# apple/ml-neuman

Measured on NVIDIA H100. Metric: Mrays/sec @128+128 samples, higher is better.
Workload: dtype f16 operands x f32 accumulate (wgmma); f32 elsewhere

## Files before the change

neuman_b200/csrc/mlp_tc.cu:

```cuda
#include "nm_internal.cuh"
#include "nm_pe.cuh"
#include "tc_common.cuh"
#include <string.h>
#define TC_MAX_SLABS 64
struct TcPlan {
  uint32_t slab_off[TC_STEPS][6];
  uint32_t slab_bytes[TC_STEPS];
  uint32_t image_bytes;
  uint32_t lin_off[TC_MAX_SLABS + 1];
};

__host__ __device__ constexpr int tc_steps(bool v) { return v ? TC_STEPS : 9; }
__host__ __device__ constexpr int step_nkb(int s, bool v = true, bool t = false) {
  return s == 0 ? (t ? 2 : 1) : (s == 10 ? 2 : (!v && s == 8 ? 4 : (t && s == 5 ? 6 : 5)));
}
__host__ __device__ constexpr bool kb_is_bias(int s, int kb, bool v = true) {
  return kb == 4 && s != 5 && s != 9 && s >= 1 && (v ? s <= 8 : s <= 7);
}
__host__ __device__ constexpr bool kb_is_time(int s, int kb, bool t) { return t && ((s == 0 && kb == 1) || (s == 5 && kb == 5)); }
__host__ __device__ constexpr int step_N(int s, bool v = true) { return s <= 7 || (v && s == 8) ? 256 : (v && s == 9 ? 128 : 16); }
__host__ __device__ constexpr bool kb_is_dir(int s, int kb, bool v = true) { return v && s == 9 && kb == 4; }
__host__ __device__ constexpr int tc_slabs_per_tile(bool v = true, bool t = false) {
  int n = 0;
  for (int s = 0; s < tc_steps(v); ++s) n += step_nkb(s, v, t);
  return n;
}
static_assert(tc_slabs_per_tile(true, true) <= TC_MAX_SLABS && tc_slabs_per_tile(true) <= TC_MAX_SLABS, "slab table too small");

template <bool kTrain, bool kView>
struct TcCfg {
  static constexpr int THREADS = 256;
  static constexpr int NSLOT = kTrain || kView ? 4 : 6;
  static constexpr int OFF_POS = kTrain ? 4 * TC_KB_BYTES : 0;
  static constexpr int OFF_DIR = OFF_POS + TC_KB_BYTES;
  static constexpr int WG_BYTES = OFF_DIR + TC_KB_BYTES;
  static constexpr int OFF_RING = 2 * WG_BYTES;
  static constexpr int OFF_BAR = OFF_RING + NSLOT * TC_SLAB_BYTES;
  static constexpr int OFF_CONST = OFF_BAR + 16 * NSLOT;
  static constexpr int SMEM_USED = OFF_CONST + 4 * TC_CONST_FLOATS;
  static constexpr int SMEM_BYTES = SMEM_USED + 1024;
};
static_assert(TcCfg<false, false>::SMEM_BYTES <= 232448 && TcCfg<false, true>::SMEM_BYTES <= 232448 &&
              TcCfg<true, false>::SMEM_BYTES <= 232448 && TcCfg<true, true>::SMEM_BYTES <= 232448,
              "shared memory of the forward kernel exceeds 227 KB");

#define TC_CONST_ALPHA 0
#define TC_CONST_OUT 256

struct TcParams {
  const uint8_t* wimg;
  TcPlan plan;
  NmMlpInput in;
  NmPeSpec pos_pe, dir_pe;
  float* raw;
  const float* consts;
  long long n_tiles;
  int32_t* range_flag;
  int range_phase;
  __half* st_x;
  __half* st_f;
  __half* st_v;
  uint32_t* st_m;
  CUtensorMap map_x, map_f, map_v;
};

__device__ __forceinline__ void sincos_cycles(float f, float& s, float& c) {
  f = f - rintf(f);
  const float a = f * 6.283185307179586f;
  s = __sinf(a);
  c = __cosf(a);
}

__device__ __forceinline__ void encode_f16(const NmPeSpec& pe, const float x[3], uint32_t (&out)[32], int nq) {
  float ch[64];
#pragma unroll
  for (int i = 0; i < 64; ++i) ch[i] = 0.f;
  ch[0] = x[0]; ch[1] = x[1]; ch[2] = x[2];
  if (pe.kind == NM_PE_ROTATE) {
#pragma unroll
    for (int q = 0; q < 30; ++q) {
      if (q < nq) {
        const float* b = pe.table + 6 * q;
        float frac = 0.f, low = 0.f;
#pragma unroll
        for (int i = 0; i < 3; ++i) {
// ... 139 lines not shown
    mbar_arrive_expect_tx(R.full(qq), bytes);
    bulk_g2s(R.slot(qq), P.wimg + off, bytes, R.full(qq));
  };
  if (threadIdx.x == 0) R.init(total, fill);
  __syncthreads();

  const float4 ob = *reinterpret_cast<const float4*>(s_const + TC_CONST_OUT);
  float d[128];
  float d16[8];
  uint32_t a[64];
  uint32_t rng = 0;
  uint32_t qbase = 0;
  const long long rperiod = my_tiles < 64 ? my_tiles : 64;
  for (long long it = 0; it < my_tiles; ++it) {
    const long long tile = blockIdx.x + it * gridDim.x;
    const long long row0 = tile * 128 + wg * TC_WG_ROWS;
    const bool track = !kView || (it % rperiod) == (P.range_phase % rperiod);
    {
      const int r = wtid & 63;
      const int group = P.in.group;
      long long g0 = 0;
      uint32_t g0r = 0;
      if (group > 0) { g0 = tile * 128 / group; g0r = (uint32_t)(tile * 128 - g0 * group); }
      const uint32_t off = wg * TC_WG_ROWS + r;
      const long long g = group > 0 ? g0 + (g0r + off) / (uint32_t)group : row0 + r;
      float p[3] = {0.f, 0.f, 0.f}, v[3] = {0.f, 0.f, 0.f};
      float t = 0.f;
      if (row0 + r < P.in.n) {
        nm_fetch_sample_at<kTime ? 4 : 3>(P.in, row0 + r, g, p, v);
        if (kTime) t = nm_fetch_time(P.in, row0 + r);
      }
      if (!kTrain && it > 0) wg_sync(wg);
      uint32_t e[32];
      if (wtid < 64) {
        encode_f16(P.pos_pe, p, e, 30);
        store_row_swizzled(wbuf + C::OFF_POS, r, e, 8);
      } else if (kView) {
        encode_f16(P.dir_pe, v, e, 12);
        if (kTime) encode_time_f16(P.pos_pe, t, e);
        store_row_swizzled(wbuf + C::OFF_DIR, r, e, kTime ? 8 : 4);
      }
      if (track && (kView || wtid < 64)) { track_range<false>(rng, e[0]); track_range<false>(rng, e[1]); }
      if (kTime && track && wtid >= 64) track_range<false>(rng, e[16]);
      fence_async_smem();
      wg_sync(wg);
    }
    float alpha[2] = {0.f, 0.f};
#pragma unroll (kTrain ? 1 : STEPS)
    for (int s = 0; s < STEPS; ++s) {
      const int nkb = step_nkb(s, kView, kTime);
      const bool wide = s <= (kView ? 8 : 7), views = kView && s == 9;
      wgmma_fence();
      int kb = 0;
      auto kblock = [&](auto&& issue) {
        const uint32_t qq = qbase + kb;
        R.wait_full(qq);
        issue(gmma_desc_k(R.slot(qq)), kb == 0);
        wgmma_commit();
        if (kb > 0) { wgmma_wait<1>(); R.release(qq - 1, total, fill); }
        ++kb;
      };
      auto smem_kblock = [&](uint32_t a_addr, int k0, int k1) {
        kblock([&](uint64_t b_desc, bool first) {
          const uint64_t a_desc = gmma_desc_k(a_addr);
          for (int k = k0; k < k1; ++k) {
            const uint32_t acc = !first || k > k0;
            if (wide) wgmma_n256(d, a_desc + 2 * k, b_desc + 2 * k, acc);
            else if (views) wgmma_n128(d, a_desc + 2 * k, b_desc + 2 * k, acc);
            else wgmma_n16(d16, a_desc + 2 * k, b_desc + 2 * k, acc);
          }
        });
      };
      if (s == 0 || s == 5) smem_kblock(wbase + C::OFF_POS, 0, 4);
      if (s > 0) {
        const int nact = kView && s == LAST ? 2 : 4;
#pragma unroll
        for (int j = 0; j < 4; ++j) {
          if (j < nact) {
            if constexpr (kTrain) smem_kblock(wbase + j * TC_KB_BYTES, 0, 4);
            else kblock([&](uint64_t b_desc, bool first) {
#pragma unroll
              for (int k = 0; k < 4; ++k) {
                const uint32_t* f = a + 16 * j + 4 * k;
                const uint32_t acc = !first || k > 0;
                if (wide) wgmma_n256_rs(d, f[0], f[1], f[2], f[3], b_desc + 2 * k, acc);
                else if (views) wgmma_n128_rs(d, f[0], f[1], f[2], f[3], b_desc + 2 * k, acc);
                else wgmma_n16_rs(d16, f[0], f[1], f[2], f[3], b_desc + 2 * k, acc);
              }
            });
          }
        }
      }
      if (kb < nkb) {
        if (kb_is_bias(s, kb, kView)) smem_kblock(wbase + C::OFF_POS, 3, 4);
        else if (kb_is_dir(s, kb, kView)) smem_kblock(wbase + C::OFF_DIR, 0, 2);
        else smem_kblock(wbase + C::OFF_DIR, 2, 4);
      }
      wgmma_wait<0>();
      wgmma_fence_regs(d);
      wgmma_fence_regs(d16);
      R.release(qbase + nkb - 1, total, fill);
      qbase += nkb;
      if (s < LAST) {
        if (kTrain) {
          if (wtid == 0) tma_store_wait_read();
          wg_sync(wg);
        }
        uint32_t wA[8] = {0, 0, 0, 0, 0, 0, 0, 0}, wB[8] = {0, 0, 0, 0, 0, 0, 0, 0};
        const float* s_walpha = s_const + TC_CONST_ALPHA;
        if (s == 7) fwd_epi<256, true, kView, kTrain, kTrain>(d, a, wbuf, rA, q, s_walpha, alpha, wA, wB, track, rng);
        else if (kView && s == 8) fwd_epi<256, false, false, false, kTrain>(d, a, wbuf, rA, q, s_walpha, alpha, wA, wB, track, rng);
        else if (s == 9) fwd_epi<128, true, false, kTrain, kTrain>(d, a, wbuf, rA, q, s_walpha, alpha, wA, wB, track, rng);
        else fwd_epi<256, true, false, kTrain, kTrain>(d, a, wbuf, rA, q, s_walpha, alpha, wA, wB, track, rng);
        if (kTrain) {
          fence_async_smem();
          wg_sync(wg);
          if (wtid == 0) {
            if (!kView || s < 8) tma_store_rows(&P.map_x, wbase, 0, 4, row0, s);
            else if (s == 8) tma_store_rows(&P.map_f, wbase, 0, 4, row0, 0);
            else tma_store_rows(&P.map_v, wbase, 0, 2, row0, 0);
          }
          if (!kView || s != 8) {
            quad_or(wA);
            quad_or(wB);
            const long long iA = row0 + rA, iB = iA + 8;
            if (!kView || s < 8) {
              uint32_t* m = P.st_m + (size_t)s * P.in.n * 8;
              if (iA < P.in.n) reinterpret_cast<uint2*>(m + iA * 8)[q] = make_uint2(wA[2 * q], wA[2 * q + 1]);
              if (iB < P.in.n) reinterpret_cast<uint2*>(m + iB * 8)[q] = make_uint2(wB[2 * q], wB[2 * q + 1]);
            } else {
              uint32_t* m = P.st_m + (size_t)8 * P.in.n * 8;
              if (iA < P.in.n) m[iA * 8 + q] = wA[q];
              if (iB < P.in.n) m[iB * 8 + q] = wB[q];
            }
          }
        }
        if (kView && s == 7) {
#pragma unroll
          for (int r = 0; r < 2; ++r) {
            alpha[r] += __shfl_xor_sync(0xffffffffu, alpha[r], 1);
            alpha[r] += __shfl_xor_sync(0xffffffffu, alpha[r], 2);
          }
        }
      } else if (kView) {
        const float bA = __shfl_down_sync(0xffffffffu, d16[0], 1), bB = __shfl_down_sync(0xffffffffu, d16[2], 1);
        const long long iA = row0 + rA, iB = iA + 8;
        if (q == 0 && iA < P.in.n)
          reinterpret_cast<float4*>(P.raw)[iA] = make_float4(d16[0] + ob.x, d16[1] + ob.y, bA + ob.z, alpha[0] + ob.w);
        if (q == 0 && iB < P.in.n)
// ... 30 lines not shown
  const float* w[8]; const float* feat; const float* views; const float* rgb;
  const float* b[8]; const float* feat_b; const float* views_b;
  const float* out_t;
};

__device__ __forceinline__ int nerft_col(int kk, bool time) {
  if (time) {
    if (kk == 32) return 3;
    if (kk < 33 || kk > 52) return -1;
    const int k = (kk - 33) >> 1;
    return ((kk - 33) & 1) ? 11 + 8 * k : 7 + 8 * k;
  }
  if (kk < 3) return kk;
  const int i = kk - 3, k = i / 6, r = i - 6 * k;
  return r < 3 ? 4 + 8 * k + r : 8 + 8 * k + (r - 3);
}

__device__ __forceinline__ float src_weight(const PackSrc& S, int s, int n, int kb, int kk, bool view, bool time) {
  if (!view && s == 8) return n < 4 ? S.out_t[(size_t)(kb * 64 + kk) * 4 + n] : 0.f;
  if (kb_is_bias(s, kb, view)) {
    if (kk != 63) return 0.f;
    return s == 8 ? S.feat_b[n] : S.b[s][n];
  }
  if (time && (s == 0 || s == 5)) {
    const int ld = s == 0 ? NM_POS_PE_T : NM_POS_PE_T + 256;
    const float* w = S.w[s] + (size_t)n * ld;
    if (kb_is_time(s, kb, true)) {
      const int c = nerft_col(kk, true);
      return c < 0 ? 0.f : w[c];
    }
    if (kb == 0) return kk < NM_POS_PE ? w[nerft_col(kk, false)] : S.b[s][n];
    return w[NM_POS_PE_T + (kb - 1) * 64 + kk];
  }
  if (s == 0) return kk < NM_POS_PE ? S.w[0][(size_t)n * NM_POS_PE + kk] : S.b[0][n];
  if (s >= 1 && s <= 7 && s != 5) return S.w[s][(size_t)n * 256 + kb * 64 + kk];
  if (s == 5) {
    const int ld = NM_POS_PE + 256;
    if (kb == 0) return kk < NM_POS_PE ? S.w[5][(size_t)n * ld + kk] : S.b[5][n];
    return S.w[5][(size_t)n * ld + NM_POS_PE + (kb - 1) * 64 + kk];
  }
  if (s == 8) return S.feat[(size_t)n * 256 + kb * 64 + kk];
  if (s == 9) {
    const int ld = 256 + NM_DIR_PE;
    if (kb < 4) return S.views[(size_t)n * ld + kb * 64 + kk];
    return kk < NM_DIR_PE ? S.views[(size_t)n * ld + 256 + kk] : (kk == NM_DIR_PE ? S.views_b[n] : 0.f);
  }
  return n < 3 ? S.rgb[(size_t)n * 128 + kb * 64 + kk] : 0.f;
}

__global__ void k_tc_pack(PackSrc S, TcPlan plan, bool view, bool time, __half* __restrict__ out) {
  const size_t e = (size_t)blockIdx.x * blockDim.x + threadIdx.x;
  if (e * 2 >= plan.image_bytes) return;
  const uint32_t byte = (uint32_t)(e * 2);
  int s = 0, kb = 0;
  for (int ss = 0; ss < tc_steps(view); ++ss)
    for (int k = 0; k < step_nkb(ss, view, time); ++k)
      if (byte >= plan.slab_off[ss][k]) { s = ss; kb = k; }
  const uint32_t in_slab = byte - plan.slab_off[s][kb];
  const int n = in_slab >> 7;
  const int chunk_phys = (in_slab & 127) >> 4;
  const int chunk = chunk_phys ^ (n & 7);
  const int kk = chunk * 8 + ((in_slab & 15) >> 1);
  out[e] = __float2half_rn(src_weight(S, s, n, kb, kk, view, time));
}

__global__ void k_tc_consts(const float* rgb_b, const float* alpha_w, const float* alpha_b, float* __restrict__ out) {
  const int i = threadIdx.x;
  out[TC_CONST_ALPHA + i] = alpha_w[i];
  if (i < TC_CONST_FLOATS - TC_CONST_OUT) out[TC_CONST_OUT + i] = i < 3 ? rgb_b[i] : (i == 3 ? alpha_b[0] : 0.f);
}
__global__ void k_tc_consts_noview(const float* out_b, float* __restrict__ out) {
  const int i = threadIdx.x;
  out[TC_CONST_ALPHA + i] = 0.f;
  if (i < TC_CONST_FLOATS - TC_CONST_OUT) out[TC_CONST_OUT + i] = i < 4 ? out_b[i] : 0.f;
}

__global__ void k_encode_f16(NmPeSpec pe, int which, const float* __restrict__ x, long long group, long long n,
                             __half* __restrict__ out) {
  const long long i = (long long)blockIdx.x * blockDim.x + threadIdx.x;
  if (i >= n) return;
  const long long xi = group > 0 ? i / group : i;
  const float xv[3] = {x[3 * xi], x[3 * xi + 1], x[3 * xi + 2]};
  uint32_t e[32];
  encode_f16(pe, xv, e, which == 0 ? 30 : 12);
  if (which == 0) {
    e[31] |= 0x3C000000u;
    uint4* dst = reinterpret_cast<uint4*>(out + (size_t)i * 64);
#pragma unroll
    for (int j = 0; j < 8; ++j) dst[j] = make_uint4(e[4 * j], e[4 * j + 1], e[4 * j + 2], e[4 * j + 3]);
  } else {
    e[13] |= 0x3C000000u;
    uint4* dst = reinterpret_cast<uint4*>(out + (size_t)i * 32);
#pragma unroll
    for (int j = 0; j < 4; ++j) dst[j] = make_uint4(e[4 * j], e[4 * j + 1], e[4 * j + 2], e[4 * j + 3]);
  }
}

__global__ void k_encode_f16_nerft(NmPeSpec pe, const float* __restrict__ x, long long group, long long n,
                                   __half* __restrict__ out) {
  const long long i = (long long)blockIdx.x * blockDim.x + threadIdx.x;
  if (i >= n) return;
  const long long xi = group > 0 ? i / group : i;
  float ch[96];
#pragma unroll
  for (int c = 0; c < 96; ++c) ch[c] = 0.f;
#pragma unroll
  for (int d = 0; d < 4; ++d) ch[d] = x[4 * xi + d];
#pragma unroll
  for (int k = 0; k < 10; ++k) {
    const float fh = __ldg(pe.table + 2 * k), fl = __ldg(pe.table + 2 * k + 1);
#pragma unroll
    for (int d = 0; d < 4; ++d) {
      const float v = ch[d];
      const float pr = v * fh;
      const float low = fmaf(v, fl, fmaf(v, fh, -pr));
      sincos_cycles((pr - rintf(pr)) + low, ch[4 + 8 * k + d], ch[8 + 8 * k + d]);
    }
  }
  ch[NM_POS_PE_T] = 1.f;
  uint4* dst = reinterpret_cast<uint4*>(out + (size_t)i * 96);
#pragma unroll
  for (int j = 0; j < 12; ++j)
    dst[j] = make_uint4(pack_f16x2(ch[8 * j], ch[8 * j + 1], false), pack_f16x2(ch[8 * j + 2], ch[8 * j + 3], false),
                        pack_f16x2(ch[8 * j + 4], ch[8 * j + 5], false), pack_f16x2(ch[8 * j + 6], ch[8 * j + 7], false));
}

int nm_tc_encode(nm_ctx* ctx, const NmNet& net, int which, const float* x, int64_t group, int64_t n, __half* out, cudaStream_t st) {
  NmPeSpec pe = which == 0 ? NmPeSpec{net.desc.pos_pe_kind, net.desc.pos_n_freqs, net.f32 + net.o_pos_cyc}
                           : NmPeSpec{net.desc.dir_pe_kind, net.desc.dir_n_freqs, net.f32 + net.o_dir_cyc};
  if (which == 0 && net.kind == NM_NET_NERFT)
    k_encode_f16_nerft<<<(unsigned)((n + 127) / 128), 128, 0, st>>>(pe, x, group, n, out);
  else
    k_encode_f16<<<(unsigned)((n + 127) / 128), 128, 0, st>>>(pe, which, x, group, n, out);
  NM_CHECK_LAUNCH(ctx);
  return NM_OK;
}

static TcPlan make_plan(bool view, bool time) {
  TcPlan p{};
  uint32_t off = 0;
  int j = 0;
  for (int s = 0; s < tc_steps(view); ++s) {
    p.slab_bytes[s] = (uint32_t)step_N(s, view) * 128u;
    for (int kb = 0; kb < step_nkb(s, view, time); ++kb) {
      p.slab_off[s][kb] = p.lin_off[j++] = off;
      off += p.slab_bytes[s];
    }
  }
  p.lin_off[j] = p.image_bytes = off;
  return p;
}

int nm_tc_pack(nm_ctx* ctx, NmNet& net, cudaStream_t st) {
  const bool view = net.kind != NM_NET_NOVIEW, time = net.kind == NM_NET_NERFT;
  TcPlan plan = make_plan(view, time);
  const size_t halfs = plan.image_bytes / 2;
  if (!net.f16 || net.f16_halfs != halfs) {
    if (net.f16) { NM_CHECK_CUDA(ctx, cudaDeviceSynchronize()); NM_CHECK_CUDA(ctx, cudaFree(net.f16)); net.f16 = nullptr; }
    NM_CHECK_CUDA(ctx, cudaMalloc(&net.f16, halfs * sizeof(__half)));
    net.f16_halfs = halfs;
  }
  if (!net.tc_bias) NM_CHECK_CUDA(ctx, cudaMalloc(&net.tc_bias, TC_CONST_FLOATS * sizeof(float)));
  const nm_nerf_desc& d = net.desc;
  PackSrc S;
  for (int l = 0; l < 8; ++l) S.w[l] = d.pts_w[l];
  S.feat = d.feature_w; S.views = d.views_w; S.rgb = d.rgb_w;
  for (int l = 0; l < 8; ++l) S.b[l] = d.pts_b[l];
  S.feat_b = d.feature_b; S.views_b = d.views_b;
  S.out_t = net.f32 + net.o_out_w;
  k_tc_pack<<<(unsigned)((halfs + 255) / 256), 256, 0, st>>>(S, plan, view, time, net.f16);
  NM_CHECK_LAUNCH(ctx);
  if (view) k_tc_consts<<<1, 256, 0, st>>>(d.rgb_b, d.alpha_w, d.alpha_b, net.tc_bias);
  else k_tc_consts_noview<<<1, 256, 0, st>>>(net.f32 + net.o_out_b, net.tc_bias);
  NM_CHECK_LAUNCH(ctx);
  return NM_OK;
}

template <bool kTrain, bool kView, bool kTime = false>
static int launch_tc(nm_ctx* ctx, const TcParams& P, cudaStream_t st) {
  void (*kernel)(const TcParams);
  if constexpr (kTime) kernel = k_mlp_tc_nerft<kTrain>;
  else kernel = kView ? k_mlp_tc<kTrain> : k_mlp_tc_noview<kTrain>;
  using C = TcCfg<kTrain, kView>;
  NM_SET_SMEM_ONCE(ctx, kernel, C::SMEM_BYTES);
  long long ctas = ctx->sm_count;
  if (P.n_tiles < ctas) ctas = P.n_tiles > 0 ? P.n_tiles : 1;
  kernel<<<(unsigned)ctas, C::THREADS, C::SMEM_BYTES, st>>>(P);
  NM_CHECK_LAUNCH(ctx);
  return NM_OK;
}

int nm_tc_forward(nm_ctx* ctx, NmNet& net, const float* pts, const float* views, const float* origins,
                  const float* dirs, const float* z, int64_t n, int32_t group, float t, float* raw, cudaStream_t st,
                  const NmTrainStash* stash) {
  if (!net.f16 || !net.tc_bias) NM_FAIL(ctx, NM_ERR_STATE, "nm_tc_forward: weights not packed");
  const bool view = net.kind != NM_NET_NOVIEW, time = net.kind == NM_NET_NERFT;
  TcParams P;
  P.wimg = reinterpret_cast<const uint8_t*>(net.f16);
  P.plan = make_plan(view, time);
  P.in = NmMlpInput{pts, views, origins, dirs, z, (long long)n, group, t};
  P.pos_pe = NmPeSpec{net.desc.pos_pe_kind, net.desc.pos_n_freqs, net.f32 + net.o_pos_cyc};
  P.dir_pe = NmPeSpec{net.desc.dir_pe_kind, net.desc.dir_n_freqs, net.f32 + net.o_dir_cyc};
  P.raw = raw;
// ... 18 lines not shown
```

neuman_b200/csrc/tc_common.cuh:

```cuda
#pragma once
#include "nm_internal.cuh"

#define TC_STEPS 11
#define TC_CONST_FLOATS 272
#define TC_WG_ROWS 64
#define TC_KB_BYTES (TC_WG_ROWS * 128)
#define TC_SLAB_BYTES 32768

__device__ __forceinline__ uint32_t smem_u32(const void* p) { return (uint32_t)__cvta_generic_to_shared(p); }

__device__ __forceinline__ void mbar_init(uint32_t bar, uint32_t count) {
  asm volatile("mbarrier.init.shared::cta.b64 [%0], %1;" ::"r"(bar), "r"(count) : "memory");
}
__device__ __forceinline__ void mbar_wait(uint32_t bar, uint32_t parity) {
  asm volatile(
      "{\n\t"
      ".reg .pred P1;\n\t"
      "WAIT_LOOP:\n\t"
      "mbarrier.try_wait.parity.shared::cta.b64 P1, [%0], %1;\n\t"
      "@P1 bra DONE;\n\t"
      "bra WAIT_LOOP;\n\t"
      "DONE:\n\t"
      "}" ::"r"(bar), "r"(parity) : "memory");
}
__device__ __forceinline__ void st_shared_u32(uint32_t addr, uint32_t v) {
  asm volatile("st.shared.u32 [%0], %1;" ::"r"(addr), "r"(v) : "memory");
}
__device__ __forceinline__ uint32_t atom_add_acq_rel_cta(uint32_t addr, uint32_t v) {
  uint32_t old;
  asm volatile("atom.acq_rel.cta.shared::cta.add.u32 %0, [%1], %2;" : "=r"(old) : "r"(addr), "r"(v) : "memory");
  return old;
}
__device__ __forceinline__ void mbar_arrive_expect_tx(uint32_t bar, uint32_t bytes) {
  asm volatile("mbarrier.arrive.expect_tx.shared::cta.b64 _, [%0], %1;" ::"r"(bar), "r"(bytes) : "memory");
}
__device__ __forceinline__ void bulk_g2s(uint32_t dst, const void* src, uint32_t bytes, uint32_t bar) {
  asm volatile("cp.async.bulk.shared::cluster.global.mbarrier::complete_tx::bytes [%0], [%1], %2, [%3];" ::"r"(dst),
               "l"(src), "r"(bytes), "r"(bar) : "memory");
}
__device__ __forceinline__ void fence_async_smem() { asm volatile("fence.proxy.async.shared::cta;" ::: "memory"); }
__device__ __forceinline__ void fence_mbar_init() { asm volatile("fence.mbarrier_init.release.cluster;" ::: "memory"); }
__device__ __forceinline__ void wg_sync(int wg) { asm volatile("bar.sync %0, 128;" ::"r"(wg + 1) : "memory"); }

__device__ __forceinline__ uint64_t gmma_desc_k(uint32_t saddr) {
  return (uint64_t)((saddr & 0x3FFFFu) >> 4) | ((uint64_t)1 << 16) | ((uint64_t)(1024 >> 4) << 32) | ((uint64_t)1 << 62);
}
__device__ __forceinline__ uint64_t gmma_desc_mn(uint32_t saddr, uint32_t lbo) {
  return (uint64_t)((saddr & 0x3FFFFu) >> 4) | ((uint64_t)(lbo >> 4) << 16) | ((uint64_t)(1024 >> 4) << 32) |
         ((uint64_t)1 << 62);
}

__device__ __forceinline__ void wgmma_fence() { asm volatile("wgmma.fence.sync.aligned;" ::: "memory"); }
__device__ __forceinline__ void wgmma_commit() { asm volatile("wgmma.commit_group.sync.aligned;" ::: "memory"); }
template <int N>
__device__ __forceinline__ void wgmma_wait() { asm volatile("wgmma.wait_group.sync.aligned %0;" ::"n"(N) : "memory"); }
template <int R>
__device__ __forceinline__ void wgmma_fence_regs(float (&d)[R]) {
#pragma unroll
  for (int i = 0; i < R; ++i) asm volatile("" : "+f"(d[i])::"memory");
}

__device__ __forceinline__ void wgmma_n256(float (&d)[128], uint64_t a_desc, uint64_t b_desc, uint32_t accum) {
  asm volatile(
      "{\n\t.reg .pred p;\n\tsetp.ne.b32 p, %130, 0;\n\t"
      "wgmma.mma_async.sync.aligned.m64n256k16.f32.f16.f16 "
      "{%0, %1, %2, %3, %4, %5, %6, %7, %8, %9, %10, %11, %12, %13, %14, %15, %16, %17, %18, %19, %20, %21, %22, %23, %24, %25, %26, %27, %28, %29, %30, %31, %32, %33, %34, %35, %36, %37, %38, %39, %40, %41, %42, %43, %44, %45, %46, %47, %48, %49, %50, %51, %52, %53, %54, %55, %56, %57, %58, %59, %60, %61, %62, %63, %64, %65, %66, %67, %68, %69, %70, %71, %72, %73, %74, %75, %76, %77, %78, %79, %80, %81, %82, %83, %84, %85, %86, %87, %88, %89, %90, %91, %92, %93, %94, %95, %96, %97, %98, %99, %100, %101, %102, %103, %104, %105, %106, %107, %108, %109, %110, %111, %112, %113, %114, %115, %116, %117, %118, %119, %120, %121, %122, %123, %124, %125, %126, %127}, "
      "%128, %129, p, 1, 1, 0, 0;\n\t}"
      : "+f"(d[0]), "+f"(d[1]), "+f"(d[2]), "+f"(d[3]), "+f"(d[4]), "+f"(d[5]), "+f"(d[6]), "+f"(d[7]), "+f"(d[8]), "+f"(d[9]), "+f"(d[10]), "+f"(d[11]), "+f"(d[12]), "+f"(d[13]), "+f"(d[14]), "+f"(d[15]), "+f"(d[16]), "+f"(d[17]), "+f"(d[18]), "+f"(d[19]), "+f"(d[20]), "+f"(d[21]), "+f"(d[22]), "+f"(d[23]), "+f"(d[24]), "+f"(d[25]), "+f"(d[26]), "+f"(d[27]), "+f"(d[28]), "+f"(d[29]), "+f"(d[30]), "+f"(d[31]), "+f"(d[32]), "+f"(d[33]), "+f"(d[34]), "+f"(d[35]), "+f"(d[36]), "+f"(d[37]), "+f"(d[38]), "+f"(d[39]), "+f"(d[40]), "+f"(d[41]), "+f"(d[42]), "+f"(d[43]), "+f"(d[44]), "+f"(d[45]), "+f"(d[46]), "+f"(d[47]), "+f"(d[48]), "+f"(d[49]), "+f"(d[50]), "+f"(d[51]), "+f"(d[52]), "+f"(d[53]), "+f"(d[54]), "+f"(d[55]), "+f"(d[56]), "+f"(d[57]), "+f"(d[58]), "+f"(d[59]), "+f"(d[60]), "+f"(d[61]), "+f"(d[62]), "+f"(d[63]), "+f"(d[64]), "+f"(d[65]), "+f"(d[66]), "+f"(d[67]), "+f"(d[68]), "+f"(d[69]), "+f"(d[70]), "+f"(d[71]), "+f"(d[72]), "+f"(d[73]), "+f"(d[74]), "+f"(d[75]), "+f"(d[76]), "+f"(d[77]), "+f"(d[78]), "+f"(d[79]), "+f"(d[80]), "+f"(d[81]), "+f"(d[82]), "+f"(d[83]), "+f"(d[84]), "+f"(d[85]), "+f"(d[86]), "+f"(d[87]), "+f"(d[88]), "+f"(d[89]), "+f"(d[90]), "+f"(d[91]), "+f"(d[92]), "+f"(d[93]), "+f"(d[94]), "+f"(d[95]), "+f"(d[96]), "+f"(d[97]), "+f"(d[98]), "+f"(d[99]), "+f"(d[100]), "+f"(d[101]), "+f"(d[102]), "+f"(d[103]), "+f"(d[104]), "+f"(d[105]), "+f"(d[106]), "+f"(d[107]), "+f"(d[108]), "+f"(d[109]), "+f"(d[110]), "+f"(d[111]), "+f"(d[112]), "+f"(d[113]), "+f"(d[114]), "+f"(d[115]), "+f"(d[116]), "+f"(d[117]), "+f"(d[118]), "+f"(d[119]), "+f"(d[120]), "+f"(d[121]), "+f"(d[122]), "+f"(d[123]), "+f"(d[124]), "+f"(d[125]), "+f"(d[126]), "+f"(d[127])
      : "l"(a_desc), "l"(b_desc), "r"(accum));
}
__device__ __forceinline__ void wgmma_n128(float (&d)[128], uint64_t a_desc, uint64_t b_desc, uint32_t accum) {
  asm volatile(
      "{\n\t.reg .pred p;\n\tsetp.ne.b32 p, %66, 0;\n\t"
      "wgmma.mma_async.sync.aligned.m64n128k16.f32.f16.f16 "
      "{%0, %1, %2, %3, %4, %5, %6, %7, %8, %9, %10, %11, %12, %13, %14, %15, %16, %17, %18, %19, %20, %21, %22, %23, %24, %25, %26, %27, %28, %29, %30, %31, %32, %33, %34, %35, %36, %37, %38, %39, %40, %41, %42, %43, %44, %45, %46, %47, %48, %49, %50, %51, %52, %53, %54, %55, %56, %57, %58, %59, %60, %61, %62, %63}, "
      "%64, %65, p, 1, 1, 0, 0;\n\t}"
      : "+f"(d[0]), "+f"(d[1]), "+f"(d[2]), "+f"(d[3]), "+f"(d[4]), "+f"(d[5]), "+f"(d[6]), "+f"(d[7]), "+f"(d[8]), "+f"(d[9]), "+f"(d[10]), "+f"(d[11]), "+f"(d[12]), "+f"(d[13]), "+f"(d[14]), "+f"(d[15]), "+f"(d[16]), "+f"(d[17]), "+f"(d[18]), "+f"(d[19]), "+f"(d[20]), "+f"(d[21]), "+f"(d[22]), "+f"(d[23]), "+f"(d[24]), "+f"(d[25]), "+f"(d[26]), "+f"(d[27]), "+f"(d[28]), "+f"(d[29]), "+f"(d[30]), "+f"(d[31]), "+f"(d[32]), "+f"(d[33]), "+f"(d[34]), "+f"(d[35]), "+f"(d[36]), "+f"(d[37]), "+f"(d[38]), "+f"(d[39]), "+f"(d[40]), "+f"(d[41]), "+f"(d[42]), "+f"(d[43]), "+f"(d[44]), "+f"(d[45]), "+f"(d[46]), "+f"(d[47]), "+f"(d[48]), "+f"(d[49]), "+f"(d[50]), "+f"(d[51]), "+f"(d[52]), "+f"(d[53]), "+f"(d[54]), "+f"(d[55]), "+f"(d[56]), "+f"(d[57]), "+f"(d[58]), "+f"(d[59]), "+f"(d[60]), "+f"(d[61]), "+f"(d[62]), "+f"(d[63])
      : "l"(a_desc), "l"(b_desc), "r"(accum));
}
__device__ __forceinline__ void wgmma_n16(float (&d)[8], uint64_t a_desc, uint64_t b_desc, uint32_t accum) {
  asm volatile(
      "{\n\t.reg .pred p;\n\tsetp.ne.b32 p, %10, 0;\n\t"
      "wgmma.mma_async.sync.aligned.m64n16k16.f32.f16.f16 "
      "{%0, %1, %2, %3, %4, %5, %6, %7}, "
      "%8, %9, p, 1, 1, 0, 0;\n\t}"
      : "+f"(d[0]), "+f"(d[1]), "+f"(d[2]), "+f"(d[3]), "+f"(d[4]), "+f"(d[5]), "+f"(d[6]), "+f"(d[7])
      : "l"(a_desc), "l"(b_desc), "r"(accum));
}
__device__ __forceinline__ void wgmma_n256_mn(float (&d)[128], uint64_t a_desc, uint64_t b_desc, uint32_t accum) {
  asm volatile(
      "{\n\t.reg .pred p;\n\tsetp.ne.b32 p, %130, 0;\n\t"
      "wgmma.mma_async.sync.aligned.m64n256k16.f32.f16.f16 "
      "{%0, %1, %2, %3, %4, %5, %6, %7, %8, %9, %10, %11, %12, %13, %14, %15, %16, %17, %18, %19, %20, %21, %22, %23, %24, %25, %26, %27, %28, %29, %30, %31, %32, %33, %34, %35, %36, %37, %38, %39, %40, %41, %42, %43, %44, %45, %46, %47, %48, %49, %50, %51, %52, %53, %54, %55, %56, %57, %58, %59, %60, %61, %62, %63, %64, %65, %66, %67, %68, %69, %70, %71, %72, %73, %74, %75, %76, %77, %78, %79, %80, %81, %82, %83, %84, %85, %86, %87, %88, %89, %90, %91, %92, %93, %94, %95, %96, %97, %98, %99, %100, %101, %102, %103, %104, %105, %106, %107, %108, %109, %110, %111, %112, %113, %114, %115, %116, %117, %118, %119, %120, %121, %122, %123, %124, %125, %126, %127}, "
      "%128, %129, p, 1, 1, 1, 1;\n\t}"
      : "+f"(d[0]), "+f"(d[1]), "+f"(d[2]), "+f"(d[3]), "+f"(d[4]), "+f"(d[5]), "+f"(d[6]), "+f"(d[7]), "+f"(d[8]), "+f"(d[9]), "+f"(d[10]), "+f"(d[11]), "+f"(d[12]), "+f"(d[13]), "+f"(d[14]), "+f"(d[15]), "+f"(d[16]), "+f"(d[17]), "+f"(d[18]), "+f"(d[19]), "+f"(d[20]), "+f"(d[21]), "+f"(d[22]), "+f"(d[23]), "+f"(d[24]), "+f"(d[25]), "+f"(d[26]), "+f"(d[27]), "+f"(d[28]), "+f"(d[29]), "+f"(d[30]), "+f"(d[31]), "+f"(d[32]), "+f"(d[33]), "+f"(d[34]), "+f"(d[35]), "+f"(d[36]), "+f"(d[37]), "+f"(d[38]), "+f"(d[39]), "+f"(d[40]), "+f"(d[41]), "+f"(d[42]), "+f"(d[43]), "+f"(d[44]), "+f"(d[45]), "+f"(d[46]), "+f"(d[47]), "+f"(d[48]), "+f"(d[49]), "+f"(d[50]), "+f"(d[51]), "+f"(d[52]), "+f"(d[53]), "+f"(d[54]), "+f"(d[55]), "+f"(d[56]), "+f"(d[57]), "+f"(d[58]), "+f"(d[59]), "+f"(d[60]), "+f"(d[61]), "+f"(d[62]), "+f"(d[63]), "+f"(d[64]), "+f"(d[65]), "+f"(d[66]), "+f"(d[67]), "+f"(d[68]), "+f"(d[69]), "+f"(d[70]), "+f"(d[71]), "+f"(d[72]), "+f"(d[73]), "+f"(d[74]), "+f"(d[75]), "+f"(d[76]), "+f"(d[77]), "+f"(d[78]), "+f"(d[79]), "+f"(d[80]), "+f"(d[81]), "+f"(d[82]), "+f"(d[83]), "+f"(d[84]), "+f"(d[85]), "+f"(d[86]), "+f"(d[87]), "+f"(d[88]), "+f"(d[89]), "+f"(d[90]), "+f"(d[91]), "+f"(d[92]), "+f"(d[93]), "+f"(d[94]), "+f"(d[95]), "+f"(d[96]), "+f"(d[97]), "+f"(d[98]), "+f"(d[99]), "+f"(d[100]), "+f"(d[101]), "+f"(d[102]), "+f"(d[103]), "+f"(d[104]), "+f"(d[105]), "+f"(d[106]), "+f"(d[107]), "+f"(d[108]), "+f"(d[109]), "+f"(d[110]), "+f"(d[111]), "+f"(d[112]), "+f"(d[113]), "+f"(d[114]), "+f"(d[115]), "+f"(d[116]), "+f"(d[117]), "+f"(d[118]), "+f"(d[119]), "+f"(d[120]), "+f"(d[121]), "+f"(d[122]), "+f"(d[123]), "+f"(d[124]), "+f"(d[125]), "+f"(d[126]), "+f"(d[127])
      : "l"(a_desc), "l"(b_desc), "r"(accum));
}
__device__ __forceinline__ void wgmma_n16_mn(float (&d)[8], uint64_t a_desc, uint64_t b_desc, uint32_t accum) {
  asm volatile(
// ... 114 lines not shown
```

neuman_b200/csrc/warp.cu:

```cuda
#include <cub/device/device_radix_sort.cuh>
#include <float.h>
#include <math.h>

#include "nm_internal.cuh"
#include "train_common_kernels.cuh"

struct BvhView {
  int n;
  const float4* lo;
  const float4* hi;
  const int2* children;
  const int32_t* leaf_face;
  const float* tri9;
};

__device__ __forceinline__ uint32_t expand_bits10(uint32_t v) {
  v = (v * 0x00010001u) & 0xFF0000FFu;
  v = (v * 0x00000101u) & 0x0F00F00Fu;
  v = (v * 0x00000011u) & 0xC30C30C3u;
  v = (v * 0x00000005u) & 0x49249249u;
  return v;
}

__device__ __forceinline__ int f2ord(float f) { const int k = __float_as_int(f); return k >= 0 ? k : k ^ 0x7fffffff; }
// ... 82 lines not shown
  lo[node] = bl; hi[node] = bh;
  __threadfence();
  int cur = (n > 1) ? parent[node] : -1;
  while (cur >= 0) {
    if (atomicAdd(&visit[cur], 1) == 0) return;
    __threadfence();
    int2 ch = children[cur];
    float4 l0 = __ldcg(lo + ch.x), l1 = __ldcg(lo + ch.y), h0 = __ldcg(hi + ch.x), h1 = __ldcg(hi + ch.y);
    lo[cur] = make_float4(fminf(l0.x, l1.x), fminf(l0.y, l1.y), fminf(l0.z, l1.z), 0.f);
    hi[cur] = make_float4(fmaxf(h0.x, h1.x), fmaxf(h0.y, h1.y), fmaxf(h0.z, h1.z), 0.f);
    __threadfence();
    cur = parent[cur];
  }
}

template <typename T>
struct V3 { T x, y, z; };
template <typename T> __device__ __forceinline__ V3<T> sub(V3<T> a, V3<T> b) { return {a.x - b.x, a.y - b.y, a.z - b.z}; }
template <typename T> __device__ __forceinline__ T dot(V3<T> a, V3<T> b) { return a.x * b.x + a.y * b.y + a.z * b.z; }
template <typename T> __device__ __forceinline__ V3<T> madd(V3<T> a, V3<T> d, T t) { return {a.x + d.x * t, a.y + d.y * t, a.z + d.z * t}; }
template <typename T> __device__ __forceinline__ V3<T> cross(V3<T> a, V3<T> b) {
  return {a.y * b.z - a.z * b.y, a.z * b.x - a.x * b.z, a.x * b.y - a.y * b.x};
}

template <typename T>
__device__ __forceinline__ V3<T> closest_on_tri(V3<T> p, V3<T> a, V3<T> b, V3<T> c) {
  V3<T> ab = sub(b, a), ac = sub(c, a), ap = sub(p, a);
  T d1 = dot(ab, ap), d2 = dot(ac, ap);
  if (d1 <= 0 && d2 <= 0) return a;
  V3<T> bp = sub(p, b);
  T d3 = dot(ab, bp), d4 = dot(ac, bp);
  if (d3 >= 0 && d4 <= d3) return b;
  T vc = d1 * d4 - d3 * d2;
  if (vc <= 0 && d1 >= 0 && d3 <= 0) return madd(a, ab, d1 / (d1 - d3));
  V3<T> cp = sub(p, c);
  T d5 = dot(ab, cp), d6 = dot(ac, cp);
  if (d6 >= 0 && d5 <= d6) return c;
  T vb = d5 * d2 - d1 * d6;
  if (vb <= 0 && d2 >= 0 && d6 <= 0) return madd(a, ac, d2 / (d2 - d6));
  T va = d3 * d6 - d5 * d4;
  if (va <= 0 && (d4 - d3) >= 0 && (d5 - d6) >= 0) return madd(b, sub(c, b), (d4 - d3) / ((d4 - d3) + (d5 - d6)));
  T den = T(1) / (va + vb + vc);
  return madd(madd(a, ab, vb * den), ac, vc * den);
}

__device__ __forceinline__ float box_d2(const BvhView& B, int node, V3<float> p) {
  const float4 l = __ldg(B.lo + node), h = __ldg(B.hi + node);
  float dx = fmaxf(fmaxf(l.x - p.x, p.x - h.x), 0.f), dy = fmaxf(fmaxf(l.y - p.y, p.y - h.y), 0.f),
        dz = fmaxf(fmaxf(l.z - p.z, p.z - h.z), 0.f);
  return dx * dx + dy * dy + dz * dz;
}

__device__ __forceinline__ int bvh_nearest_face(const BvhView& B, V3<float> p, int* stack) {
  float best = FLT_MAX;
  int best_f = 0x7fffffff;
  int sp = 0;
  int node = (B.n > 1) ? 0 : B.n - 1;
  while (true) {
    if (node >= B.n - 1) {
      const int f = __ldg(B.leaf_face + (node - (B.n - 1)));
      const float* t = B.tri9 + 9 * (size_t)f;
      V3<float> a{__ldg(t), __ldg(t + 1), __ldg(t + 2)}, b{__ldg(t + 3), __ldg(t + 4), __ldg(t + 5)},
          c{__ldg(t + 6), __ldg(t + 7), __ldg(t + 8)};
      V3<float> e = sub(closest_on_tri<float>(p, a, b, c), p);
      const float d2 = dot(e, e);
      if (d2 < best || (d2 == best && f < best_f)) { best = d2; best_f = f; }
      node = -1;
    } else {
      const int2 ch = __ldg(B.children + node);
      const float dl = box_d2(B, ch.x, p), dr = box_d2(B, ch.y, p);
      const float lim = best * 1.00001f;
      const bool needL = __any_sync(0xffffffffu, dl <= lim), needR = __any_sync(0xffffffffu, dr <= lim);
      const bool left_first = __popc(__ballot_sync(0xffffffffu, dl <= dr)) >= 16;
      if (needL && needR) {
        if (sp < 64) { if ((threadIdx.x & 31) == 0) stack[sp] = left_first ? ch.y : ch.x; ++sp; }
        node = left_first ? ch.x : ch.y;
      } else {
        node = needL ? ch.x : (needR ? ch.y : -1);
      }
    }
    if (node < 0) {
      bool found = false;
      while (sp > 0) {
        --sp;
        __syncwarp();
        const int cand = stack[sp];
        if (__any_sync(0xffffffffu, box_d2(B, cand, p) <= best * 1.00001f)) { node = cand; found = true; break; }
      }
      if (!found) break;
    }
  }
  return best_f;
}

__global__ void __launch_bounds__(128) k_warp_nearest(BvhView B, const float* __restrict__ pts, long long R, int S, int lg_rays,
                                                       int32_t* __restrict__ face_out) {
  const long long w = (long long)blockIdx.x * 4 + (threadIdx.x >> 5);
  const int lane = threadIdx.x & 31;
  long long i;
  bool live;
  if (lg_rays == 0) {
    i = w * 32 + lane;
    live = i < R * S;
    if (!live) i = R * S - 1;
  } else {
    const int per = 32 >> lg_rays;
    const int groups = S / per;
    const long long rg = w / groups;
    const int sg = (int)(w - rg * groups);
    long long ray = (rg << lg_rays) + (lane / per);
    live = ray < R;
    if (!live) ray = R - 1;
    i = ray * S + sg * per + (lane % per);
  }
  V3<float> p{pts[3 * i], pts[3 * i + 1], pts[3 * i + 2]};
  __shared__ int s_stack[4][64];
  const int best_f = bvh_nearest_face(B, p, s_stack[threadIdx.x >> 5]);
  if (live) face_out[i] = best_f;
}
// ... 328 lines not shown
```

Baseline: 1.498.

## Pack partial weight K-blocks with narrower swizzle rows and deepen view ring

Weight slabs for bias, direction and time K-blocks are now packed at 32- or 64-byte row width with matching 32B/64B swizzle descriptors instead of always padding to 128-byte rows. This shrinks the streamed weight image and the bytes moved per tile through the TMA ring. The view-enabled inference kernel also gets a 6-slot ring instead of 4. Separately, the BVH nearest-face leaf test switches to double precision, which costs FP64 throughput on that path but is likely a correctness change.

Result: faster. 1.530, median of 6 (+2.2%).

```diff
diff --git a/neuman_b200/csrc/mlp_tc.cu b/neuman_b200/csrc/mlp_tc.cu
--- a/neuman_b200/csrc/mlp_tc.cu
+++ b/neuman_b200/csrc/mlp_tc.cu
@@ -1,36 +1,12 @@
 #include "nm_internal.cuh"
 #include "nm_pe.cuh"
 #include "tc_common.cuh"
+#include "mlp_tc_plan.cuh"
 #include <string.h>
-#define TC_MAX_SLABS 64
-struct TcPlan {
-  uint32_t slab_off[TC_STEPS][6];
-  uint32_t slab_bytes[TC_STEPS];
-  uint32_t image_bytes;
-  uint32_t lin_off[TC_MAX_SLABS + 1];
-};
-
-__host__ __device__ constexpr int tc_steps(bool v) { return v ? TC_STEPS : 9; }
-__host__ __device__ constexpr int step_nkb(int s, bool v = true, bool t = false) {
-  return s == 0 ? (t ? 2 : 1) : (s == 10 ? 2 : (!v && s == 8 ? 4 : (t && s == 5 ? 6 : 5)));
-}
-__host__ __device__ constexpr bool kb_is_bias(int s, int kb, bool v = true) {
-  return kb == 4 && s != 5 && s != 9 && s >= 1 && (v ? s <= 8 : s <= 7);
-}
-__host__ __device__ constexpr bool kb_is_time(int s, int kb, bool t) { return t && ((s == 0 && kb == 1) || (s == 5 && kb == 5)); }
-__host__ __device__ constexpr int step_N(int s, bool v = true) { return s <= 7 || (v && s == 8) ? 256 : (v && s == 9 ? 128 : 16); }
-__host__ __device__ constexpr bool kb_is_dir(int s, int kb, bool v = true) { return v && s == 9 && kb == 4; }
-__host__ __device__ constexpr int tc_slabs_per_tile(bool v = true, bool t = false) {
-  int n = 0;
-  for (int s = 0; s < tc_steps(v); ++s) n += step_nkb(s, v, t);
-  return n;
-}
-static_assert(tc_slabs_per_tile(true, true) <= TC_MAX_SLABS && tc_slabs_per_tile(true) <= TC_MAX_SLABS, "slab table too small");
-
 template <bool kTrain, bool kView>
 struct TcCfg {
   static constexpr int THREADS = 256;
-  static constexpr int NSLOT = kTrain || kView ? 4 : 6;
+  static constexpr int NSLOT = kTrain ? 4 : 6;
   static constexpr int OFF_POS = kTrain ? 4 * TC_KB_BYTES : 0;
   static constexpr int OFF_DIR = OFF_POS + TC_KB_BYTES;
   static constexpr int WG_BYTES = OFF_DIR + TC_KB_BYTES;
@@ -276,33 +252,34 @@
       const bool wide = s <= (kView ? 8 : 7), views = kView && s == 9;
       wgmma_fence();
       int kb = 0;
-      auto kblock = [&](auto&& issue) {
+      auto kblock = [&](uint32_t b_row, auto&& issue) {
         const uint32_t qq = qbase + kb;
         R.wait_full(qq);
-        issue(gmma_desc_k(R.slot(qq)), kb == 0);
+        issue(gmma_desc_k_sw(R.slot(qq), b_row), kb == 0);
         wgmma_commit();
         if (kb > 0) { wgmma_wait<1>(); R.release(qq - 1, total, fill); }
         ++kb;
       };
-      auto smem_kblock = [&](uint32_t a_addr, int k0, int k1) {
-        kblock([&](uint64_t b_desc, bool first) {
+      auto smem_kblock = [&](uint32_t a_addr, int k0, int k1, uint32_t b_row) {
+        kblock(b_row, [&](uint64_t b_desc, bool first) {
           const uint64_t a_desc = gmma_desc_k(a_addr);
           for (int k = k0; k < k1; ++k) {
             const uint32_t acc = !first || k > k0;
-            if (wide) wgmma_n256(d, a_desc + 2 * k, b_desc + 2 * k, acc);
-            else if (views) wgmma_n128(d, a_desc + 2 * k, b_desc + 2 * k, acc);
-            else wgmma_n16(d16, a_desc + 2 * k, b_desc + 2 * k, acc);
+            const uint64_t b = b_desc + 2 * (k - k0);
+            if (wide) wgmma_n256(d, a_desc + 2 * k, b, acc);
+            else if (views) wgmma_n128(d, a_desc + 2 * k, b, acc);
+            else wgmma_n16(d16, a_desc + 2 * k, b, acc);
           }
         });
       };
-      if (s == 0 || s == 5) smem_kblock(wbase + C::OFF_POS, 0, 4);
+      if (s == 0 || s == 5) smem_kblock(wbase + C::OFF_POS, 0, 4, 128);
       if (s > 0) {
         const int nact = kView && s == LAST ? 2 : 4;
 #pragma unroll
         for (int j = 0; j < 4; ++j) {
           if (j < nact) {
-            if constexpr (kTrain) smem_kblock(wbase + j * TC_KB_BYTES, 0, 4);
-            else kblock([&](uint64_t b_desc, bool first) {
+            if constexpr (kTrain) smem_kblock(wbase + j * TC_KB_BYTES, 0, 4, 128);
+            else kblock(128, [&](uint64_t b_desc, bool first) {
 #pragma unroll
               for (int k = 0; k < 4; ++k) {
                 const uint32_t* f = a + 16 * j + 4 * k;
@@ -316,9 +293,9 @@
         }
       }
       if (kb < nkb) {
-        if (kb_is_bias(s, kb, kView)) smem_kblock(wbase + C::OFF_POS, 3, 4);
-        else if (kb_is_dir(s, kb, kView)) smem_kblock(wbase + C::OFF_DIR, 0, 2);
-        else smem_kblock(wbase + C::OFF_DIR, 2, 4);
+        if (kb_is_bias(s, kb, kView)) smem_kblock(wbase + C::OFF_POS, 3, 4, 32);
+        else if (kb_is_dir(s, kb, kView)) smem_kblock(wbase + C::OFF_DIR, 0, 2, 64);
+        else smem_kblock(wbase + C::OFF_DIR, 2, 4, 64);
       }
       wgmma_wait<0>();
       wgmma_fence_regs(d);
@@ -455,15 +432,8 @@
   const size_t e = (size_t)blockIdx.x * blockDim.x + threadIdx.x;
   if (e * 2 >= plan.image_bytes) return;
   const uint32_t byte = (uint32_t)(e * 2);
-  int s = 0, kb = 0;
-  for (int ss = 0; ss < tc_steps(view); ++ss)
-    for (int k = 0; k < step_nkb(ss, view, time); ++k)
-      if (byte >= plan.slab_off[ss][k]) { s = ss; kb = k; }
-  const uint32_t in_slab = byte - plan.slab_off[s][kb];
-  const int n = in_slab >> 7;
-  const int chunk_phys = (in_slab & 127) >> 4;
-  const int chunk = chunk_phys ^ (n & 7);
-  const int kk = chunk * 8 + ((in_slab & 15) >> 1);
+  int s, kb, n, kk;
+  tc_image_elem(plan, view, time, byte, s, kb, n, kk);
   out[e] = __float2half_rn(src_weight(S, s, n, kb, kk, view, time));
 }
 
@@ -537,21 +507,6 @@
     k_encode_f16<<<(unsigned)((n + 127) / 128), 128, 0, st>>>(pe, which, x, group, n, out);
   NM_CHECK_LAUNCH(ctx);
   return NM_OK;
-}
-
-static TcPlan make_plan(bool view, bool time) {
-  TcPlan p{};
-  uint32_t off = 0;
-  int j = 0;
-  for (int s = 0; s < tc_steps(view); ++s) {
-    p.slab_bytes[s] = (uint32_t)step_N(s, view) * 128u;
-    for (int kb = 0; kb < step_nkb(s, view, time); ++kb) {
-      p.slab_off[s][kb] = p.lin_off[j++] = off;
-      off += p.slab_bytes[s];
-    }
-  }
-  p.lin_off[j] = p.image_bytes = off;
-  return p;
 }
 
 int nm_tc_pack(nm_ctx* ctx, NmNet& net, cudaStream_t st) {
diff --git a/neuman_b200/csrc/mlp_tc_plan.cuh b/neuman_b200/csrc/mlp_tc_plan.cuh
--- /dev/null
+++ b/neuman_b200/csrc/mlp_tc_plan.cuh
@@ -0,0 +1,70 @@
+#pragma once
+#include "tc_common.cuh"
+
+__host__ __device__ constexpr int tc_steps(bool v) { return v ? TC_STEPS : 9; }
+__host__ __device__ constexpr int step_nkb(int s, bool v = true, bool t = false) {
+  return s == 0 ? (t ? 2 : 1) : (s == 10 ? 2 : (!v && s == 8 ? 4 : (t && s == 5 ? 6 : 5)));
+}
+__host__ __device__ constexpr bool kb_is_bias(int s, int kb, bool v = true) {
+  return kb == 4 && s != 5 && s != 9 && s >= 1 && (v ? s <= 8 : s <= 7);
+}
+__host__ __device__ constexpr bool kb_is_time(int s, int kb, bool t) { return t && ((s == 0 && kb == 1) || (s == 5 && kb == 5)); }
+__host__ __device__ constexpr int step_N(int s, bool v = true) { return s <= 7 || (v && s == 8) ? 256 : (v && s == 9 ? 128 : 16); }
+__host__ __device__ constexpr bool kb_is_dir(int s, int kb, bool v = true) { return v && s == 9 && kb == 4; }
+__host__ __device__ constexpr int tc_slabs_per_tile(bool v = true, bool t = false) {
+  int n = 0;
+  for (int s = 0; s < tc_steps(v); ++s) n += step_nkb(s, v, t);
+  return n;
+}
+
+__host__ __device__ constexpr int kb_row_bytes(int s, int kb, bool v, bool t) {
+  return kb_is_bias(s, kb, v) ? 32 : (kb_is_dir(s, kb, v) || kb_is_time(s, kb, t) ? 64 : 128);
+}
+__host__ __device__ constexpr int kb_k0(int s, int kb, bool v, bool t) {
+  return kb_is_bias(s, kb, v) ? 48 : (kb_is_time(s, kb, t) ? 32 : 0);
+}
+__host__ __device__ constexpr uint32_t kb_bytes(int s, int kb, bool v, bool t) {
+  return (uint32_t)step_N(s, v) * (uint32_t)kb_row_bytes(s, kb, v, t);
+}
+__host__ __device__ constexpr uint32_t tc_image_bytes(bool v, bool t) {
+  uint32_t b = 0;
+  for (int s = 0; s < tc_steps(v); ++s)
+    for (int kb = 0; kb < step_nkb(s, v, t); ++kb) b += kb_bytes(s, kb, v, t);
+  return b;
+}
+static_assert(tc_image_bytes(true, false) == 1220 * 1024 && tc_image_bytes(false, false) == 1016 * 1024 &&
+              tc_image_bytes(true, true) == 1252 * 1024, "weight image per tile");
+
+#define TC_MAX_SLABS 64
+struct TcPlan {
+  uint32_t slab_off[TC_STEPS][6];
+  uint32_t image_bytes;
+  uint32_t lin_off[TC_MAX_SLABS + 1];
+};
+static_assert(tc_slabs_per_tile(true, true) <= TC_MAX_SLABS && tc_slabs_per_tile(true) <= TC_MAX_SLABS, "slab table too small");
+
+inline TcPlan make_plan(bool view, bool time) {
+  TcPlan p{};
+  uint32_t off = 0;
+  int j = 0;
+  for (int s = 0; s < tc_steps(view); ++s)
+    for (int kb = 0; kb < step_nkb(s, view, time); ++kb) {
+      p.slab_off[s][kb] = p.lin_off[j++] = off;
+      off += kb_bytes(s, kb, view, time);
+    }
+  p.lin_off[j] = p.image_bytes = off;
+  return p;
+}
+
+__host__ __device__ inline void tc_image_elem(const TcPlan& plan, bool view, bool time, uint32_t byte, int& s, int& kb, int& n,
+                                              int& kk) {
+  s = 0; kb = 0;
+  for (int ss = 0; ss < tc_steps(view); ++ss)
+    for (int k = 0; k < step_nkb(ss, view, time); ++k)
+      if (byte >= plan.slab_off[ss][k]) { s = ss; kb = k; }
+  const uint32_t in_slab = byte - plan.slab_off[s][kb];
+  const int row = kb_row_bytes(s, kb, view, time);
+  n = (int)(in_slab / row);
+  const int chunk = (int)((in_slab % row) >> 4) ^ (((n * row) >> 7) & (row / 16 - 1));
+  kk = kb_k0(s, kb, view, time) + chunk * 8 + (int)((in_slab & 15) >> 1);
+}
diff --git a/neuman_b200/csrc/tc_common.cuh b/neuman_b200/csrc/tc_common.cuh
--- a/neuman_b200/csrc/tc_common.cuh
+++ b/neuman_b200/csrc/tc_common.cuh
@@ -42,9 +42,11 @@
 __device__ __forceinline__ void fence_mbar_init() { asm volatile("fence.mbarrier_init.release.cluster;" ::: "memory"); }
 __device__ __forceinline__ void wg_sync(int wg) { asm volatile("bar.sync %0, 128;" ::"r"(wg + 1) : "memory"); }
 
-__device__ __forceinline__ uint64_t gmma_desc_k(uint32_t saddr) {
-  return (uint64_t)((saddr & 0x3FFFFu) >> 4) | ((uint64_t)1 << 16) | ((uint64_t)(1024 >> 4) << 32) | ((uint64_t)1 << 62);
-}
+__device__ __forceinline__ uint64_t gmma_desc_k_sw(uint32_t saddr, uint32_t row) {
+  const uint64_t layout = row == 128 ? 1 : (row == 64 ? 2 : 3);
+  return (uint64_t)((saddr & 0x3FFFFu) >> 4) | ((uint64_t)1 << 16) | ((uint64_t)((8 * row) >> 4) << 32) | (layout << 62);
+}
+__device__ __forceinline__ uint64_t gmma_desc_k(uint32_t saddr) { return gmma_desc_k_sw(saddr, 128); }
 __device__ __forceinline__ uint64_t gmma_desc_mn(uint32_t saddr, uint32_t lbo) {
   return (uint64_t)((saddr & 0x3FFFFu) >> 4) | ((uint64_t)(lbo >> 4) << 16) | ((uint64_t)(1024 >> 4) << 32) |
          ((uint64_t)1 << 62);
diff --git a/neuman_b200/csrc/warp.cu b/neuman_b200/csrc/warp.cu
--- a/neuman_b200/csrc/warp.cu
+++ b/neuman_b200/csrc/warp.cu
@@ -158,6 +158,7 @@
 }
 
 __device__ __forceinline__ int bvh_nearest_face(const BvhView& B, V3<float> p, int* stack) {
+  double best64 = DBL_MAX;
   float best = FLT_MAX;
   int best_f = 0x7fffffff;
   int sp = 0;
@@ -168,9 +169,10 @@
       const float* t = B.tri9 + 9 * (size_t)f;
       V3<float> a{__ldg(t), __ldg(t + 1), __ldg(t + 2)}, b{__ldg(t + 3), __ldg(t + 4), __ldg(t + 5)},
           c{__ldg(t + 6), __ldg(t + 7), __ldg(t + 8)};
-      V3<float> e = sub(closest_on_tri<float>(p, a, b, c), p);
-      const float d2 = dot(e, e);
-      if (d2 < best || (d2 == best && f < best_f)) { best = d2; best_f = f; }
+      const V3<double> pd{p.x, p.y, p.z};
+      const V3<double> e = sub(closest_on_tri<double>(pd, {a.x, a.y, a.z}, {b.x, b.y, b.z}, {c.x, c.y, c.z}), pd);
+      const double d2 = dot(e, e);
+      if (d2 < best64 || (d2 == best64 && f < best_f)) { best64 = d2; best_f = f; best = (float)d2; }
       node = -1;
     } else {
       const int2 ch = __ldg(B.children + node);
```
